# kjenike/panagram

Measured on AMD Instinct MI355X. Metric: anchored k-mers/sec building pan-kmer bitmap, higher is better.
Workload: dtype u64

## Files before the change

### panagram_amd/csrc/pg_api.hip

```cpp
#include "../../include/panagram_hip.h"
#include "pg_kernels.h"
#include "pg_guard.h"

#include <algorithm>
#include <atomic>
#include <condition_variable>
#include <cmath>
#include <cstdarg>
#include <cstdio>
#include <cstdlib>
#include <cstring>
#include <memory>
#include <mutex>
#include <string>
#include <system_error>
#include <thread>
#include <vector>

using namespace pg;

static thread_local std::string g_err;

static int fail(int code, const char *fmt, ...) {
    char buf[512];
    va_list ap;
    va_start(ap, fmt);
    vsnprintf(buf, sizeof buf, fmt, ap);
    va_end(ap);
    g_err = buf;
    return code;
}

#define HIP_TRY(expr)                                                                          \
    do {                                                                                       \
        hipError_t e_ = (expr);                                                                \
        if (e_ != hipSuccess)                                                                  \
            return fail(PG_E_HIP, "%s failed: %s (%s:%d)", #expr, hipGetErrorString(e_), __FILE__, __LINE__); \
    } while (0)

extern "C" const char *pg_last_error(void) { return g_err.c_str(); }
int pg_set_error(int code, const char *msg) {
    g_err = msg ? msg : "";
    return code;
}
extern "C" const char *pg_version(void) { return "panagram_hip 0.2 gfx950"; }
extern "C" uint32_t pg_tile_positions(void) { return (uint32_t)PROBE_TILE; }

struct pg_ctx {
    int device;
    hipStream_t own_stream;
    hipStream_t stream;
    hipStream_t aux_stream;
    std::atomic<int> refs{0};
    bool dead = false;
    struct DfSet {
        uint8_t *d_slots[2] = {nullptr, nullptr}, *d_packed[2] = {nullptr, nullptr}, *h_slots[2] = {nullptr, nullptr};
        uint32_t *d_sizes[2] = {nullptr, nullptr}, *d_offs[2] = {nullptr, nullptr}, *h_sizes[2] = {nullptr, nullptr};
        uint32_t *d_crc = nullptr, *d_hist = nullptr;
        void *d_code = nullptr;
        bool ready = false, busy = false;
    } df[4];
    std::mutex df_mu;
    std::condition_variable df_cv;
    struct RowBuf {
        uint8_t *p;
        uint64_t cap;
    };
    std::vector<RowBuf> row_cache;
    std::mutex row_mu;
};

struct SubHost {
    SubTable d;
    uint64_t count;
};

struct pg_table {
    pg_ctx *ctx;
    int k, ngenomes, ndbs;
    uint32_t m;
    bool m_pinned = false;
    uint32_t cosched = 0;
    uint64_t expected = 0;
    double load0 = 0.375;
    uint64_t first_len = 0;
    uint64_t max_len = 0;
    std::vector<SubHost> subs;
    unsigned long long *d_counters;
    unsigned long long *h_counters = nullptr;
    uint32_t *d_tile0 = nullptr;
    size_t tile0_cap = 0;
    double spill = 0;
    std::atomic<int> refs{0};
    bool dead = false;
    std::mutex write_mu;
};
#define TABLE_WRITER(t) std::lock_guard<std::mutex> writer_guard_((t)->write_mu)

struct pg_seqset {
    pg_ctx *ctx;
    uint32_t n;
    std::vector<SeqDesc> desc;
    uint64_t total_words;
    uint64_t *d_seqw;
    uint32_t *d_nmw;
    uint32_t *d_has_n;
    SeqDesc *d_desc;
    void *d_stage;
    size_t stage_cap;
    std::vector<std::string> names;
    std::atomic<int> refs{0};
    bool dead = false;
};

struct pg_result {
    pg_ctx *ctx;
    pg_table *tbl;
    const pg_seqset *seqs;
    uint32_t N;
    int k;
    uint32_t flags;
    uint32_t lowres_step = 100;
    std::vector<AnchorDesc> ad;
    std::vector<uint64_t> nrows100;
    AnchorDesc *d_ad;
    uint32_t *d_tile_contig;
    uint32_t *d_sched = nullptr;
    std::vector<uint32_t> sched_bounds;
    uint32_t ntiles;
    uint8_t *d_out1;
    uint64_t out1_bytes;
    uint64_t out1_cap = 0;
    uint8_t *d_out100;
    uint64_t out100_bytes;
    uint32_t *d_bins;
    uint64_t total_bins;
    unsigned long long *d_colsums;
    hipEvent_t ev[4];
    bool ev_ok, ev_epi;
    bool rows_valid = false;
    struct EvSet {
        hipEvent_t e[4];
        bool probe, epi;
    };
    std::vector<EvSet> ev_hist, ev_free;
    struct Chunk {
        uint32_t s0, s1, r0, nr, tiles;
    };
    std::vector<Chunk> chunks;
    uint2 *d_ranges = nullptr;
    bool chunks_ready = false;
    std::vector<hipEvent_t> chunk_ev;
    size_t hist_skip = 0;
    double probe_ms_sum = 0, epi_ms_sum = 0;
    uint32_t probe_runs = 0, epi_runs = 0;
    int fuse_state = 0;
    uint32_t *d_tile_hist = nullptr, *d_tile_cs = nullptr;
    uint2 *d_small = nullptr;
    uint32_t n_small = 0, small_tiles = 0;
    uint32_t fused_runs = 0;
};
static constexpr size_t EV_RING = 128;

static constexpr uint32_t MAX_PROBE = 512;
static constexpr double GROW_AT = 0.55;
#ifndef PG_INLINE_LAYOUT
#define PG_INLINE_LAYOUT 1
#endif
static constexpr double TARGET_LOAD = 0.375;
static constexpr double HARD_LOAD = 0.85;

static int use_device(const pg_ctx *c) {
    HIP_TRY(hipSetDevice(c->device));
    return PG_OK;
}

extern "C" int pg_ctx_create(int device_id, pg_ctx **out) {
    PG_API_BEGIN
    if (!out) return fail(PG_E_INVALID, "pg_ctx_create: out is NULL");
    int n = 0;
    hipError_t e = hipGetDeviceCount(&n);
    if (e != hipSuccess || n == 0)
        return fail(PG_E_HIP, "no HIP device visible (%s); libpanagram_hip has no CPU fallback",
                    e == hipSuccess ? "device count 0" : hipGetErrorString(e));
    if (device_id < 0 || device_id >= n) return fail(PG_E_INVALID, "device %d out of range (0..%d)", device_id, n - 1);
    HIP_TRY(hipSetDevice(device_id));
    pg_ctx *c = new pg_ctx();
    c->device = device_id;
    hipError_t se = hipStreamCreateWithFlags(&c->own_stream, hipStreamNonBlocking);
    if (se != hipSuccess) {
        delete c;
        return fail(PG_E_HIP, "hipStreamCreate failed: %s", hipGetErrorString(se));
    }
    c->stream = c->own_stream;
    se = hipStreamCreateWithFlags(&c->aux_stream, hipStreamNonBlocking);
    if (se != hipSuccess) {
        hipStreamDestroy(c->own_stream);
        delete c;
        return fail(PG_E_HIP, "hipStreamCreate failed: %s", hipGetErrorString(se));
    }
    hipError_t pe = preload_table_kernels();
    if (pe == hipSuccess) pe = preload_anchor_kernels();
    if (pe == hipSuccess) pe = preload_rows_kernels();
    if (pe == hipSuccess) pe = preload_deflate_kernels();
    if (pe != hipSuccess) {
        hipStreamDestroy(c->aux_stream);
        hipStreamDestroy(c->own_stream);
        delete c;
        return fail(PG_E_HIP, "loading the gfx950 kernels failed: %s (is this an MI355X?)", hipGetErrorString(pe));
    }
    *out = c;
    return PG_OK;
    PG_API_END
}

static void df_free_buffers(pg_ctx::DfSet &d);
static void ctx_free(pg_ctx *c) {
    hipSetDevice(c->device);
    hipStreamSynchronize(c->stream);
    hipStreamSynchronize(c->aux_stream);
    for (auto &b : c->row_cache) hipFree(b.p);
    c->row_cache.clear();
    for (auto &d : c->df) df_free_buffers(d);
    hipStreamDestroy(c->aux_stream);
    hipStreamDestroy(c->own_stream);
    delete c;
}
static void ctx_release(pg_ctx *c) {
    if (--c->refs == 0 && c->dead) ctx_free(c);
}

static constexpr uint64_t ROW_CACHE_MIN = 1ull << 30;
static void row_cache_trim(pg_ctx *c) {
    std::lock_guard<std::mutex> lk(c->row_mu);
    for (auto &b : c->row_cache) hipFree(b.p);
    c->row_cache.clear();
}
static hipError_t row_alloc(pg_ctx *c, uint64_t bytes, uint8_t **out, uint64_t *cap) {
    {
        std::lock_guard<std::mutex> lk(c->row_mu);
        for (size_t i = 0; i < c->row_cache.size(); ++i)
            if (c->row_cache[i].cap >= bytes && c->row_cache[i].cap <= 2 * bytes) {
                *out = c->row_cache[i].p;
                *cap = c->row_cache[i].cap;
                c->row_cache.erase(c->row_cache.begin() + (long)i);
                return hipSuccess;
            }
    }
    hipError_t e = hipMalloc(reinterpret_cast<void **>(out), bytes);
    if (e != hipSuccess) {
        (void)hipGetLastError();
        row_cache_trim(c);
        e = hipMalloc(reinterpret_cast<void **>(out), bytes);
    }
    *cap = bytes;
    return e;
}
static void row_free(pg_ctx *c, uint8_t *p, uint64_t cap) {
    if (!p) return;
    if (cap >= ROW_CACHE_MIN && !c->dead) {
        std::lock_guard<std::mutex> lk(c->row_mu);
        if (c->row_cache.size() < 2) {
            c->row_cache.push_back({p, cap});
            return;
        }
    }
    hipFree(p);
}

extern "C" int pg_host_alloc(pg_ctx *c, uint64_t nbytes, void **out) {
    PG_API_BEGIN
    if (!c || !out) return fail(PG_E_INVALID, "pg_host_alloc: NULL argument");
    if (int r = use_device(c)) return r;
    *out = nullptr;
    hipError_t e = hipHostMalloc(out, std::max<uint64_t>(nbytes, 1), hipHostMallocDefault);
    if (e != hipSuccess) {
        (void)hipGetLastError();
        *out = nullptr;
        return fail(PG_E_HIP, "hipHostMalloc(%llu bytes) failed: %s", (unsigned long long)nbytes, hipGetErrorString(e));
    }
    return PG_OK;
    PG_API_END
}

extern "C" int pg_host_free(pg_ctx *c, void *p) {
    PG_API_BEGIN
    if (!c) return fail(PG_E_INVALID, "ctx is NULL");
    if (!p) return PG_OK;
    if (int r = use_device(c)) return r;
    HIP_TRY(hipHostFree(p));
    return PG_OK;
    PG_API_END
// ... 1672 lines not shown
        return fail(PG_E_HIP, "pg_seqset_slice: %s", hipGetErrorString(e));
    }
    *out = s;
    return PG_OK;
    PG_API_END
}

extern "C" uint32_t pg_seqset_ncontigs(const pg_seqset *s) { return s ? s->n : 0; }

extern "C" int pg_seqset_contig(const pg_seqset *s, uint32_t idx, const char **name, uint64_t *len) {
    PG_API_BEGIN
    if (!s) return fail(PG_E_INVALID, "seqset is NULL");
    if (idx >= s->n) return fail(PG_E_INVALID, "contig %u out of range", idx);
    if (name) *name = idx < s->names.size() ? s->names[idx].c_str() : "";
    if (len) *len = s->desc[idx].len;
    return PG_OK;
    PG_API_END
}

extern "C" int pg_seqset_describe(const pg_seqset *s, uint64_t *lens, char *names, uint64_t names_cap, uint64_t *names_bytes) {
    PG_API_BEGIN
    if (!s) return fail(PG_E_INVALID, "seqset is NULL");
    uint64_t need = 0;
    for (uint32_t i = 0; i < s->n; ++i) {
        if (lens) lens[i] = s->desc[i].len;
        need += (i < s->names.size() ? s->names[i].size() : 0) + 1;
    }
    if (names_bytes) *names_bytes = need;
    if (names) {
        if (names_cap < need) return fail(PG_E_INVALID, "pg_seqset_describe: %llu bytes of names, room for %llu", (unsigned long long)need, (unsigned long long)names_cap);
        char *p = names;
        for (uint32_t i = 0; i < s->n; ++i) {
            if (i < s->names.size()) {
                memcpy(p, s->names[i].data(), s->names[i].size());
                p += s->names[i].size();
            }
            *p++ = 0;
        }
    }
    return PG_OK;
    PG_API_END
}

extern "C" int pg_seqset_unpack(const pg_seqset *s, uint32_t idx, char *out) {
    PG_API_BEGIN
    if (!s || !out) return fail(PG_E_INVALID, "pg_seqset_unpack: NULL argument");
    if (idx >= s->n) return fail(PG_E_INVALID, "contig %u out of range", idx);
    if (int r = use_device(s->ctx)) return r;
    const SeqDesc &d = s->desc[idx];
    const uint64_t nw = (d.len + 31) / 32;
    std::vector<uint64_t> w(nw);
    std::vector<uint32_t> nm(nw);
    if (nw) {
        HIP_TRY(hipMemcpyAsync(w.data(), s->d_seqw + d.seq_off, nw * 8, hipMemcpyDeviceToHost, s->ctx->stream));
        HIP_TRY(hipMemcpyAsync(nm.data(), s->d_nmw + d.seq_off, nw * 4, hipMemcpyDeviceToHost, s->ctx->stream));
        HIP_TRY(hipStreamSynchronize(s->ctx->stream));
    }
    for (uint64_t i = 0; i < d.len; ++i)
        out[i] = ((nm[i >> 5] >> (i & 31)) & 1u) ? 'N' : "ACGT"[(w[i >> 5] >> (2 * (i & 31))) & 3u];
    return PG_OK;
    PG_API_END
}

extern "C" uint64_t pg_seqset_total_kmers(const pg_seqset *s, int k) {
    uint64_t t = 0;
    if (s)
        for (auto &d : s->desc)
            if (d.len >= (uint64_t)k) t += d.len - k + 1;
    return t;
}

static TableDesc make_desc(const pg_table *t) {
    TableDesc T;
    memset(&T, 0, sizeof T);
    T.nsub = (uint32_t)t->subs.size();
    for (uint32_t i = 0; i < T.nsub; ++i) T.sub[i] = t->subs[i].d;
    T.ndbs = t->ndbs;
    T.k = t->k;
    T.ngenomes = t->ngenomes;
    return T;
}

struct ResultGeom {
    uint32_t lowres_step = 100;
    uint64_t max_bin_len = 200000;
    uint32_t min_bin_count = 100;
};

static int result_create(pg_ctx *ctx, pg_table *t, int k, uint32_t N, const pg_seqset *sq, uint32_t flags,
                         const ResultGeom &geo, pg_result **out) {
    if (ctx != sq->ctx) return fail(PG_E_INVALID, "table / context and seqset belong to different contexts");
    if (geo.lowres_step < 1 || geo.max_bin_len < 1 || geo.min_bin_count < 1)
        return fail(PG_E_INVALID, "lowres_step, max_bin_len and min_bin_count must be >= 1");
    if (int r = use_device(ctx)) return r;
    const uint32_t nbytes = (N + 7) / 8;
    pg_result *r = new pg_result();
    r->ctx = ctx;
    r->tbl = t;
    r->seqs = sq;
    r->N = N;
    r->k = k;
    if (t) ++t->refs;
    else ++ctx->refs;
    ++const_cast<pg_seqset *>(sq)->refs;
    r->flags = flags;
    r->lowres_step = geo.lowres_step;
    r->d_ad = nullptr;
    r->d_tile_contig = nullptr;
    r->d_out1 = r->d_out100 = nullptr;
    r->d_bins = nullptr;
    r->d_colsums = nullptr;
    r->ev_ok = r->ev_epi = false;
    for (auto &e : r->ev) e = nullptr;
    uint64_t o1 = 0, o100 = 0, bins = 0, tiles = 0;
    std::vector<uint32_t> tile_contig;
    for (uint32_t c = 0; c < sq->n; ++c) {
        const uint64_t len = sq->desc[c].len;
        const uint64_t nk = len >= (uint64_t)k ? len - k + 1 : 0;
        if (nk > 0xFFFFFFF0ull) {
            pg_result_destroy(r);
            return fail(PG_E_INVALID, "contig %u has %llu k-mers; contigs must stay below 2^32 (as in KMC)", c, (unsigned long long)nk);
        }
        AnchorDesc a;
        a.nkmers = (uint32_t)nk;
        uint64_t binlen = geo.max_bin_len;
        if (nk / binlen < geo.min_bin_count) binlen = nk / geo.min_bin_count;
        if (binlen == 0) binlen = 1;
        a.binlen = (uint32_t)binlen;
        a.nbins = (uint32_t)((nk + binlen - 1) / binlen);
        a.out_off = o1;
        a.out100_off = o100;
        a.bin_off = bins;
        a.tile0 = (uint32_t)tiles;
        const uint64_t n100 = (nk + geo.lowres_step - 1) / geo.lowres_step;
        r->nrows100.push_back(n100);
        o1 += (nk * nbytes + 15) & ~15ull;
        o100 += n100 * nbytes;
        bins += a.nbins;
        const uint64_t nt = (nk + PROBE_TILE - 1) / PROBE_TILE;
        for (uint64_t i = 0; i < nt; ++i) tile_contig.push_back(c);
        tiles += nt;
        r->ad.push_back(a);
    }
    if (tiles > 0x7FFFFFFFull) {
        pg_result_destroy(r);
        return fail(PG_E_INVALID, "too many tiles in one launch");
    }
    r->ntiles = (uint32_t)tiles;
    r->out1_bytes = o1;
    r->out100_bytes = o100;
    r->total_bins = bins;
    hipStream_t st = ctx->stream;
    hipError_t e;
    if ((e = hipMalloc(reinterpret_cast<void **>(&r->d_ad), std::max<size_t>(1, r->ad.size()) * sizeof(AnchorDesc))) == hipSuccess &&
        (e = hipMalloc(reinterpret_cast<void **>(&r->d_tile_contig), std::max<size_t>(1, tile_contig.size()) * 4)) == hipSuccess &&
        (e = row_alloc(ctx, (flags & PG_ANCHOR_COLUMNS_ONLY) ? 16 : std::max<uint64_t>(16, o1) + 16, &r->d_out1, &r->out1_cap)) == hipSuccess &&
        (e = hipMalloc(reinterpret_cast<void **>(&r->d_out100), std::max<uint64_t>(16, o100))) == hipSuccess &&
        (e = hipMalloc(reinterpret_cast<void **>(&r->d_bins), std::max<uint64_t>(1, bins) * (N + 1) * 4)) == hipSuccess &&
        (e = hipMalloc(reinterpret_cast<void **>(&r->d_colsums), std::max<size_t>(1, r->ad.size()) * N * 8)) == hipSuccess) {
        if (!r->ad.empty())
            e = hipMemcpyAsync(r->d_ad, r->ad.data(), r->ad.size() * sizeof(AnchorDesc), hipMemcpyHostToDevice, st);
        if (e == hipSuccess && !tile_contig.empty())
            e = hipMemcpyAsync(r->d_tile_contig, tile_contig.data(), tile_contig.size() * 4, hipMemcpyHostToDevice, st);
        if (e == hipSuccess && !t) e = hipMemsetAsync(r->d_out1, 0, std::max<uint64_t>(16, o1), st);
        if (e == hipSuccess) e = hipStreamSynchronize(st);
    }
    if (e != hipSuccess) {
        pg_result_destroy(r);
        return fail(PG_E_HIP, "result allocation failed: %s", hipGetErrorString(e));
    }
    *out = r;
    return PG_OK;
}

extern "C" int pg_result_create(pg_table *t, const pg_seqset *sq, uint32_t flags, pg_result **out) {
    PG_API_BEGIN
    if (!t || !sq || !out) return fail(PG_E_INVALID, "pg_result_create: NULL argument");
    return result_create(t->ctx, t, t->k, (uint32_t)t->ngenomes, sq, flags, ResultGeom(), out);
    PG_API_END
}

extern "C" int pg_result_create_ex(pg_table *t, const pg_seqset *sq, uint32_t flags, uint32_t lowres_step,
                                   uint64_t max_bin_len, uint32_t min_bin_count, pg_result **out) {
    PG_API_BEGIN
    if (!t || !sq || !out) return fail(PG_E_INVALID, "pg_result_create_ex: NULL argument");
    ResultGeom g;
    g.lowres_step = lowres_step;
    g.max_bin_len = max_bin_len;
    g.min_bin_count = min_bin_count;
    return result_create(t->ctx, t, t->k, (uint32_t)t->ngenomes, sq, flags, g, out);
    PG_API_END
}

extern "C" int pg_result_create_rows(pg_ctx *ctx, int k, int ngenomes, const pg_seqset *sq, uint32_t flags,
                                     uint32_t lowres_step, uint64_t max_bin_len, uint32_t min_bin_count, pg_result **out) {
    PG_API_BEGIN
    if (!ctx || !sq || !out) return fail(PG_E_INVALID, "pg_result_create_rows: NULL argument");
    if (k < 1 || k > 32) return fail(PG_E_INVALID, "k=%d unsupported (1..32)", k);
    if (ngenomes < 1) return fail(PG_E_INVALID, "ngenomes must be >= 1");
    ResultGeom g;
    g.lowres_step = lowres_step;
    g.max_bin_len = max_bin_len;
    g.min_bin_count = min_bin_count;
    return result_create(ctx, nullptr, k, (uint32_t)ngenomes, sq, flags | PG_ANCHOR_ROWS_ONLY, g, out);
    PG_API_END
}

extern "C" int pg_result_destroy(pg_result *r) {
    PG_API_BEGIN
    if (!r) return PG_OK;
    hipSetDevice(r->ctx->device);
    hipStreamSynchronize(r->ctx->stream);
    hipStreamSynchronize(r->ctx->aux_stream);
    hipFree(r->d_ad);
    hipFree(r->d_tile_contig);
    row_free(r->ctx, r->d_out1, r->out1_cap);
    hipFree(r->d_out100);
    hipFree(r->d_bins);
    hipFree(r->d_colsums);
    if (r->d_sched) hipFree(r->d_sched);
    if (r->d_ranges) hipFree(r->d_ranges);
    if (r->d_tile_hist) hipFree(r->d_tile_hist);
    if (r->d_tile_cs) hipFree(r->d_tile_cs);
    if (r->d_small) hipFree(r->d_small);
    for (auto e : r->chunk_ev) hipEventDestroy(e);
    for (auto *v : {&r->ev_hist, &r->ev_free})
        for (auto &s : *v)
            for (auto &e : s.e)
                if (e) hipEventDestroy(e);
    pg_table *t = r->tbl;
    pg_ctx *c = r->ctx;
    pg_seqset *sq = const_cast<pg_seqset *>(r->seqs);
    delete r;
    if (t) table_release(t);
    else ctx_release(c);
    seqset_release(sq);
    return PG_OK;
    PG_API_END
}

static int build_chunks(pg_result *r, const uint32_t *sched) {
    r->chunks.clear();
    r->chunks_ready = true;
    if (r->d_ranges) {
        hipFree(r->d_ranges);
        r->d_ranges = nullptr;
    }
    const char *env = getenv("PG_RUN_CHUNKS");
    const uint32_t nbytes = (r->N + 7) / 8;
    uint32_t K = env ? (uint32_t)atoi(env) : ((nbytes == 8 && r->ntiles >= (4u << 20)) ? 16u : 1u);
    const char *mt = getenv("PG_CHUNK_MIN_TILES");
    K = std::min(K, r->ntiles / std::max(1u, mt ? (uint32_t)atoi(mt) : 32768u));
    if (K < 2) return PG_OK;
    std::vector<uint2> ranges;
    for (uint32_t c = 0; c < K; ++c) {
        pg_result::Chunk ch;
        ch.s0 = (uint32_t)((uint64_t)r->ntiles * c / K);
        ch.s1 = (uint32_t)((uint64_t)r->ntiles * (c + 1) / K);
        ch.r0 = (uint32_t)ranges.size();
        ch.tiles = ch.s1 - ch.s0;
        if (!sched) {
            ranges.push_back(make_uint2(ch.s0, ch.s1));
        } else {
            std::vector<uint2> runs;
            for (uint32_t i = ch.s0; i < ch.s1; ++i) {
                if (!runs.empty() && runs.back().y == sched[i]) ++runs.back().y;
                else runs.push_back(make_uint2(sched[i], sched[i] + 1));
            }
            std::sort(runs.begin(), runs.end(), [](const uint2 &a, const uint2 &b) { return a.x < b.x; });
            for (const uint2 &u : runs) {
                if (ranges.size() > ch.r0 && ranges.back().y == u.x) ranges.back().y = u.y;
                else ranges.push_back(u);
            }
        }
        ch.nr = (uint32_t)ranges.size() - ch.r0;
        if (ch.nr > 512) {
            r->chunks.clear();
            return PG_OK;
        }
        r->chunks.push_back(ch);
    }
    HIP_TRY(hipMalloc(reinterpret_cast<void **>(&r->d_ranges), ranges.size() * sizeof(uint2)));
    HIP_TRY(hipMemcpy(r->d_ranges, ranges.data(), ranges.size() * sizeof(uint2), hipMemcpyHostToDevice));
    while (r->chunk_ev.size() < r->chunks.size()) {
        hipEvent_t e;
        HIP_TRY(hipEventCreateWithFlags(&e, hipEventDisableTiming));
        r->chunk_ev.push_back(e);
    }
    return PG_OK;
}

static int coschedule(pg_result *r, const uint32_t *contig_group, uint32_t piece_tiles, const uint32_t *range_first,
                      uint32_t nranges, const uint32_t *contig_class = nullptr) {
    if (int e = use_device(r->ctx)) return e;
    hipStream_t st = r->ctx->stream;
    HIP_TRY(hipStreamSynchronize(st));
    HIP_TRY(hipStreamSynchronize(r->ctx->aux_stream));
    if (r->d_sched) {
        hipFree(r->d_sched);
        r->d_sched = nullptr;
    }
    r->sched_bounds.clear();
    r->chunks.clear();
    r->chunks_ready = false;
    if (!contig_group || r->ntiles == 0) return PG_OK;
    const bool auto_piece = piece_tiles == 0;
    const size_t nc = r->ad.size();
    std::vector<uint32_t> firsts;
    if (range_first && nranges) {
        for (uint32_t i = 0; i < nranges; ++i) {
            if (range_first[i] >= nc || (i && range_first[i] <= range_first[i - 1]) || (!i && range_first[0] != 0))
                return fail(PG_E_INVALID, "pg_result_coschedule_ranges: range starts must begin at contig 0 and increase");
            firsts.push_back(range_first[i]);
        }
    } else {
        firsts.push_back(0);
    }
    firsts.push_back((uint32_t)nc);
    struct Piece {
        double at;
        uint32_t g, first;
    };
    std::vector<uint32_t> sched;
    sched.reserve(r->ntiles);
    std::vector<std::vector<uint32_t>> members;
    if (contig_class) {
        std::vector<std::pair<uint32_t, uint32_t>> byclass;
        for (size_t c = 0; c < nc; ++c) byclass.emplace_back(contig_class[c], (uint32_t)c);
        std::stable_sort(byclass.begin(), byclass.end(), [](auto &x, auto &y) { return x.first < y.first; });
        for (size_t i = 0; i < byclass.size(); ++i) {
            if (i == 0 || byclass[i].first != byclass[i - 1].first) members.emplace_back();
            members.back().push_back(byclass[i].second);
        }
        r->sched_bounds.push_back(0);
    } else {
        for (size_t ri = 0; ri + 1 < firsts.size(); ++ri) {
            members.emplace_back();
            for (uint32_t c = firsts[ri]; c < firsts[ri + 1]; ++c) members.back().push_back(c);
            r->sched_bounds.push_back(r->ad[firsts[ri]].tile0);
        }
    }
    for (const auto &mem : members) {
        uint32_t ngroups = 0;
        for (uint32_t c : mem) ngroups = std::max(ngroups, contig_group[c] + 1);
        std::vector<std::vector<uint32_t>> tiles(ngroups);
        for (uint32_t c : mem) {
            const uint32_t nt = (uint32_t)(((uint64_t)r->ad[c].nkmers + PROBE_TILE - 1) / PROBE_TILE);
            for (uint32_t i = 0; i < nt; ++i) tiles[contig_group[c]].push_back(r->ad[c].tile0 + i);
        }
        if (auto_piece) piece_tiles = ngroups <= 32 ? 64u : std::max(8u, 512u / ngroups);
        std::vector<Piece> pieces;
        for (uint32_t g = 0; g < ngroups; ++g) {
            const size_t np = (tiles[g].size() + piece_tiles - 1) / piece_tiles;
            for (size_t i = 0; i < np; ++i) pieces.push_back({(double)i / (double)np, g, (uint32_t)(i * piece_tiles)});
        }
        std::stable_sort(pieces.begin(), pieces.end(), [](const Piece &x, const Piece &y) { return x.at < y.at; });
        for (const Piece &p : pieces) {
            const size_t end = std::min<size_t>(tiles[p.g].size(), (size_t)p.first + piece_tiles);
            for (size_t i = p.first; i < end; ++i) sched.push_back(tiles[p.g][i]);
        }
    }
    r->sched_bounds.push_back(r->ntiles);
    if (sched.size() != r->ntiles) return fail(PG_E_INVALID, "internal: schedule does not cover the tiles");
    HIP_TRY(hipMalloc(reinterpret_cast<void **>(&r->d_sched), (size_t)r->ntiles * 4));
    HIP_TRY(hipMemcpyAsync(r->d_sched, sched.data(), (size_t)r->ntiles * 4, hipMemcpyHostToDevice, st));
    HIP_TRY(hipStreamSynchronize(st));
    if (!(r->flags & PG_ANCHOR_ROWS_ONLY)) return build_chunks(r, sched.data());
    return PG_OK;
}

extern "C" int pg_result_coschedule(pg_result *r, const uint32_t *contig_group, uint32_t piece_tiles) {
    PG_API_BEGIN
    if (!r) return fail(PG_E_INVALID, "result is NULL");
    return coschedule(r, contig_group, piece_tiles, nullptr, 0);
    PG_API_END
}

extern "C" int pg_result_coschedule_classes(pg_result *r, const uint32_t *contig_group, const uint32_t *contig_class,
                                            uint32_t piece_tiles) {
    PG_API_BEGIN
    if (!r) return fail(PG_E_INVALID, "result is NULL");
    if (contig_group && !contig_class) return fail(PG_E_INVALID, "pg_result_coschedule_classes: contig_class is NULL");
    return coschedule(r, contig_group, piece_tiles, nullptr, 0, contig_class);
    PG_API_END
}

extern "C" int pg_result_coschedule_ranges(pg_result *r, const uint32_t *contig_group, uint32_t piece_tiles,
                                           const uint32_t *range_first_contig, uint32_t nranges) {
    PG_API_BEGIN
    if (!r) return fail(PG_E_INVALID, "result is NULL");
    return coschedule(r, contig_group, piece_tiles, range_first_contig, nranges);
    PG_API_END
}

static int enqueue_epilogue(pg_result *r, hipStream_t st) {
    const uint32_t N = r->N;
    HIP_TRY(hipMemsetAsync(r->d_bins, 0, std::max<uint64_t>(1, r->total_bins) * (N + 1) * 4, st));
    HIP_TRY(hipMemsetAsync(r->d_colsums, 0, std::max<size_t>(1, r->ad.size()) * N * 8, st));
    const uint32_t kflags = (r->flags & PG_ANCHOR_COLSUMS) | (r->lowres_step == 100 ? 0u : 2u);
    HIP_TRY(launch_rows_epilogue(st, N, r->d_ad, r->d_tile_contig, r->ntiles, r->d_out1, r->d_out100, r->d_bins,
                                 r->d_colsums, kflags));
    if (r->lowres_step != 100)
        HIP_TRY(launch_lowres(st, N, r->d_ad, r->d_tile_contig, r->ntiles, r->d_out1, r->d_out100, r->lowres_step));
    return PG_OK;
}

static bool fuse_enabled() {
    const char *e = getenv("PG_FUSE_STATS");
    return e && *e == '1';
}
static bool fuse_table_ok(const TableDesc &T, uint32_t N) {
    return T.nsub == 1 && T.ngenomes == N && !(T.sub[0].layout == LAYOUT_SLOTS && T.sub[0].slots != 8);
}
static int prepare_fuse(pg_result *r, const TableDesc &T) {
    if (r->fuse_state) return PG_OK;
    r->fuse_state = -1;
    const uint32_t nbytes = (r->N + 7) / 8;
    if (!fuse_rows_ok(nbytes) || !fuse_table_ok(T, r->N)) return PG_OK;
    std::vector<uint2> small;
    uint64_t small_tiles = 0, fused_tiles = 0;
    for (const AnchorDesc &a : r->ad) {
        const uint32_t nt = (uint32_t)(((uint64_t)a.nkmers + PROBE_TILE - 1) / PROBE_TILE);
        if (!nt) continue;
        if (a.binlen >= (uint32_t)PROBE_TILE) {
            fused_tiles += nt;
            continue;
        }
        small_tiles += nt;
        if (!small.empty() && small.back().y == a.tile0) small.back().y = a.tile0 + nt;
        else small.push_back(make_uint2(a.tile0, a.tile0 + nt));
    }
    if (!fused_tiles || small.size() > 16384) return PG_OK;
    const size_t hb = (size_t)r->ntiles * fuse_hist_words(r->N) * 4, cb = (size_t)r->ntiles * fuse_cs_words(r->N) * 4;
    if (hipMalloc(reinterpret_cast<void **>(&r->d_tile_hist), hb) != hipSuccess || hipMalloc(reinterpret_cast<void **>(&r->d_tile_cs), cb) != hipSuccess ||
        (!small.empty() && hipMalloc(reinterpret_cast<void **>(&r->d_small), small.size() * sizeof(uint2)) != hipSuccess)) {
        (void)hipGetLastError();
        if (r->d_tile_hist) hipFree(r->d_tile_hist);
        if (r->d_tile_cs) hipFree(r->d_tile_cs);
        r->d_tile_hist = r->d_tile_cs = nullptr;
        return PG_OK;
    }
    if (!small.empty()) HIP_TRY(hipMemcpy(r->d_small, small.data(), small.size() * sizeof(uint2), hipMemcpyHostToDevice));
    r->n_small = (uint32_t)small.size();
    r->small_tiles = (uint32_t)small_tiles;
    r->fuse_state = 1;
    return PG_OK;
}
static FuseArgs fuse_args(const pg_result *r) {
    FuseArgs fa;
    fa.out100 = r->lowres_step == 100 ? r->d_out100 : nullptr;
    fa.tile_hist = r->d_tile_hist;
    fa.tile_cs = r->d_tile_cs;
    fa.ngenomes = r->N;
    fa.hw = fuse_hist_words(r->N);
    fa.csw = fuse_cs_words(r->N);
    return fa;
}
static int enqueue_fused_epilogue(pg_result *r, hipStream_t st, const FuseArgs &fa) {
    const uint32_t N = r->N;
    HIP_TRY(hipMemsetAsync(r->d_bins, 0, std::max<uint64_t>(1, r->total_bins) * (N + 1) * 4, st));
    HIP_TRY(hipMemsetAsync(r->d_colsums, 0, std::max<size_t>(1, r->ad.size()) * N * 8, st));
    HIP_TRY(launch_tile_reduce(st, fa, r->d_ad, r->d_tile_contig, r->ntiles, r->d_bins, r->d_colsums, (r->flags & PG_ANCHOR_COLSUMS) ? 1u : 0u));
    const uint32_t kflags = (r->flags & PG_ANCHOR_COLSUMS) | (r->lowres_step == 100 ? 0u : 2u);
    if (r->n_small)
        HIP_TRY(launch_rows_epilogue(st, N, r->d_ad, r->d_tile_contig, r->ntiles, r->d_out1, r->d_out100, r->d_bins, r->d_colsums, kflags,
                                     r->d_small, r->n_small, r->small_tiles));
    if (r->lowres_step != 100)
        HIP_TRY(launch_lowres(st, N, r->d_ad, r->d_tile_contig, r->ntiles, r->d_out1, r->d_out100, r->lowres_step));
    return PG_OK;
}

static int join_result(pg_result *r) {
    if (r->ev_epi) HIP_TRY(hipStreamWaitEvent(r->ctx->stream, r->ev[3], 0));
    return PG_OK;
}

static int fold_timing(pg_result *r, const pg_result::EvSet &s) {
    HIP_TRY(hipEventSynchronize(s.e[s.epi ? 3 : 1]));
    float a = 0, b = 0;
    if (s.probe) {
        HIP_TRY(hipEventElapsedTime(&a, s.e[0], s.e[1]));
        r->probe_ms_sum += a;
        ++r->probe_runs;
    }
    if (s.epi) {
        HIP_TRY(hipEventElapsedTime(&b, s.e[2], s.e[3]));
        r->epi_ms_sum += b;
        ++r->epi_runs;
    }
    return PG_OK;
}

static int next_events(pg_result *r, bool probe) {
    if (r->ev_hist.size() >= EV_RING) {
        if (r->hist_skip) --r->hist_skip;
        else if (int e = fold_timing(r, r->ev_hist.front())) return e;
        r->ev_free.push_back(r->ev_hist.front());
        r->ev_hist.erase(r->ev_hist.begin());
    }
    pg_result::EvSet s;
    if (!r->ev_free.empty()) {
        s = r->ev_free.back();
        r->ev_free.pop_back();
    } else {
        for (auto &e : s.e) {
            e = nullptr;
            HIP_TRY(hipEventCreate(&e));
        }
    }
    s.probe = probe;
    s.epi = false;
    r->ev_hist.push_back(s);
    for (int i = 0; i < 4; ++i) r->ev[i] = s.e[i];
    return PG_OK;
}

static int contig_tiles(const pg_result *r, uint32_t first, uint32_t n, uint32_t *t0, uint32_t *nt) {
    if ((uint64_t)first + n > r->ad.size()) return fail(PG_E_INVALID, "contigs %u..%u out of range (the result has %zu)", first, first + n, r->ad.size());
    if (n == 0) {
        *t0 = *nt = 0;
        return PG_OK;
    }
    const AnchorDesc &a = r->ad[first], &z = r->ad[first + n - 1];
    *t0 = a.tile0;
    *nt = z.tile0 + (uint32_t)(((uint64_t)z.nkmers + PROBE_TILE - 1) / PROBE_TILE) - a.tile0;
    return PG_OK;
}

static bool sched_covers(const pg_result *r, uint32_t t0, uint32_t nt) {
    if (!r->d_sched) return false;
    const auto &b = r->sched_bounds;
    return std::binary_search(b.begin(), b.end(), t0) && std::binary_search(b.begin(), b.end(), t0 + nt);
}

static int run_chunks(pg_result *r, const TableDesc &T) {
    hipStream_t st = r->ctx->stream, aux = r->ctx->aux_stream;
    if (const char *e = getenv("PG_CHUNK_SAME_STREAM"); e && *e == '1') aux = st;
    const uint32_t N = r->N;
    const uint32_t kflags = (r->flags & PG_ANCHOR_COLSUMS) | (r->lowres_step == 100 ? 0u : 2u);
    HIP_TRY(hipEventRecord(r->ev[0], st));
    for (size_t c = 0; c < r->chunks.size(); ++c) {
        const pg_result::Chunk &ch = r->chunks[c];
        HIP_TRY(launch_anchor(st, T, r->seqs->d_seqw, r->seqs->d_nmw, r->seqs->d_has_n, r->seqs->d_desc, r->d_ad, r->d_tile_contig,
                              r->d_sched, ch.s0, ch.s1 - ch.s0, r->d_out1, r->out1_bytes, 0));
        HIP_TRY(hipEventRecord(r->chunk_ev[c], st));
        HIP_TRY(hipStreamWaitEvent(aux, r->chunk_ev[c], 0));
        if (c == 0) {
            HIP_TRY(hipEventRecord(r->ev[2], aux));
            HIP_TRY(hipMemsetAsync(r->d_bins, 0, std::max<uint64_t>(1, r->total_bins) * (N + 1) * 4, aux));
            HIP_TRY(hipMemsetAsync(r->d_colsums, 0, std::max<size_t>(1, r->ad.size()) * N * 8, aux));
        }
        HIP_TRY(launch_rows_epilogue(aux, N, r->d_ad, r->d_tile_contig, r->ntiles, r->d_out1, r->d_out100, r->d_bins, r->d_colsums,
                                     kflags, r->d_ranges + ch.r0, ch.nr, ch.tiles));
    }
    HIP_TRY(hipEventRecord(r->ev[1], st));
    if (r->lowres_step != 100)
        HIP_TRY(launch_lowres(aux, N, r->d_ad, r->d_tile_contig, r->ntiles, r->d_out1, r->d_out100, r->lowres_step));
    HIP_TRY(hipEventRecord(r->ev[3], aux));
    r->ev_ok = r->ev_epi = true;
    r->ev_hist.back().epi = true;
    return PG_OK;
}

static int anchor_run(pg_result *r, uint32_t tile_base, uint32_t ntiles, bool whole, uint32_t columns_width = 0,
                      void *d_columns = nullptr) {
    pg_table *t = r->tbl;
    if (!t) return fail(PG_E_INVALID, "this result is a rows container (pg_result_create_rows): it has no table to probe");
    if (int e = use_device(r->ctx)) return e;
    hipStream_t st = r->ctx->stream, aux = r->ctx->aux_stream;
    if (int e = join_result(r)) return e;
    if (int e = next_events(r, true)) return e;
    TableDesc T = make_desc(t);
    const bool stats = whole && !columns_width && !(r->flags & PG_ANCHOR_ROWS_ONLY);
    bool fuse = false;
    if (stats && fuse_enabled()) {
        if (int e = prepare_fuse(r, T)) return e;
        fuse = r->fuse_state == 1 && fuse_table_ok(T, r->N);
    }
    if (stats && !fuse) {
        if (!r->chunks_ready)
            if (int e = build_chunks(r, nullptr)) return e;
        if (r->chunks.size() > 1) return run_chunks(r, T);
    }
    const FuseArgs fa = fuse_args(r);
    HIP_TRY(hipEventRecord(r->ev[0], st));
    HIP_TRY(launch_anchor(st, T, r->seqs->d_seqw, r->seqs->d_nmw, r->seqs->d_has_n, r->seqs->d_desc, r->d_ad,
                          r->d_tile_contig, sched_covers(r, tile_base, ntiles) ? r->d_sched : nullptr, tile_base, ntiles,
                          columns_width ? static_cast<uint8_t *>(d_columns) : r->d_out1, r->out1_bytes, columns_width, fuse ? &fa : nullptr));
    HIP_TRY(hipEventRecord(r->ev[1], st));
    r->ev_ok = true;
    r->ev_epi = false;
    if (stats) {
        HIP_TRY(hipStreamWaitEvent(aux, r->ev[1], 0));
        HIP_TRY(hipEventRecord(r->ev[2], aux));
        if (fuse) {
            if (int e = enqueue_fused_epilogue(r, aux, fa)) return e;
            ++r->fused_runs;
        } else if (int e = enqueue_epilogue(r, aux)) return e;
        HIP_TRY(hipEventRecord(r->ev[3], aux));
        r->ev_epi = true;
        r->ev_hist.back().epi = true;
    }
    return PG_OK;
}

extern "C" int pg_anchor_run(pg_result *r) {
    PG_API_BEGIN
    if (!r) return fail(PG_E_INVALID, "result is NULL");
    if (r->flags & PG_ANCHOR_COLUMNS_ONLY) return fail(PG_E_INVALID, "a PG_ANCHOR_COLUMNS_ONLY result has no rows: use pg_anchor_run_columns_range");
    return anchor_run(r, 0, r->ntiles, true);
    PG_API_END
}

extern "C" int pg_anchor_run_range(pg_result *r, uint32_t first_contig, uint32_t ncontigs) {
    PG_API_BEGIN
    if (!r) return fail(PG_E_INVALID, "result is NULL");
    if (r->flags & PG_ANCHOR_COLUMNS_ONLY) return fail(PG_E_INVALID, "a PG_ANCHOR_COLUMNS_ONLY result has no rows: use pg_anchor_run_columns_range");
    if (!(r->flags & PG_ANCHOR_ROWS_ONLY)) return fail(PG_E_INVALID, "pg_anchor_run_range needs a PG_ANCHOR_ROWS_ONLY result");
    uint32_t t0, nt;
    if (int e = contig_tiles(r, first_contig, ncontigs, &t0, &nt)) return e;
    return anchor_run(r, t0, nt, false);
    PG_API_END
}

extern "C" int pg_result_columns_direct(const pg_result *r, uint32_t width) {
    PG_API_BEGIN
    if (!r || !r->tbl) return 0;
    const pg_table *t = r->tbl;
    return t->subs.size() == 1 && t->subs[0].d.layout == LAYOUT_SLOTS && t->subs[0].d.W == 1 && t->subs[0].d.slots == 8 &&
           t->ngenomes <= 8 && width <= 8 && (int)width >= t->ngenomes;
    PG_API_END
}

extern "C" int pg_anchor_run_columns_range(pg_result *r, uint32_t first_contig, uint32_t ncontigs, uint32_t width, void *d_dst) {
    PG_API_BEGIN
    if (!r || !d_dst) return fail(PG_E_INVALID, "pg_anchor_run_columns_range: NULL argument");
    if (!pg_result_columns_direct(r, width))
        return fail(PG_E_INVALID, "pg_anchor_run_columns_range: needs a table of up to 8 genomes (8-slot lines) and width in ngenomes..8");
    uint32_t t0, nt;
    if (int e = contig_tiles(r, first_contig, ncontigs, &t0, &nt)) return e;
    return anchor_run(r, t0, nt, false, width, d_dst);
    PG_API_END
}

extern "C" int pg_result_timing(pg_result *r, float *probe_ms, float *epilogue_ms) {
    PG_API_BEGIN
    if (!r) return fail(PG_E_INVALID, "result is NULL");
    if (!r->ev_ok) return fail(PG_E_INVALID, "pg_anchor_run has not been called on this result");
    if (int e = use_device(r->ctx)) return e;
    HIP_TRY(hipEventSynchronize(r->ev[r->ev_epi ? 3 : 1]));
    float a = 0, b = 0;
    HIP_TRY(hipEventElapsedTime(&a, r->ev[0], r->ev[1]));
    if (r->ev_epi) HIP_TRY(hipEventElapsedTime(&b, r->ev[2], r->ev[3]));
    if (probe_ms) *probe_ms = a;
    if (epilogue_ms) *epilogue_ms = b;
    return PG_OK;
    PG_API_END
}

extern "C" int pg_result_fused_runs(const pg_result *r, uint32_t *n) {
    PG_API_BEGIN
    if (!r || !n) return fail(PG_E_INVALID, "pg_result_fused_runs: NULL argument");
    *n = r->fused_runs;
    return PG_OK;
    PG_API_END
}

extern "C" int pg_result_timing_reset(pg_result *r) {
    PG_API_BEGIN
    if (!r) return fail(PG_E_INVALID, "result is NULL");
    while (r->ev_hist.size() > 1) {
        r->ev_free.push_back(r->ev_hist.front());
        r->ev_hist.erase(r->ev_hist.begin());
    }
    r->hist_skip = r->ev_hist.size();
    r->probe_ms_sum = r->epi_ms_sum = 0;
    r->probe_runs = r->epi_runs = 0;
    return PG_OK;
    PG_API_END
}

extern "C" int pg_result_timing_mean(pg_result *r, double *probe_ms, double *epilogue_ms, uint32_t *nruns) {
    PG_API_BEGIN
    if (!r) return fail(PG_E_INVALID, "result is NULL");
    if (int e = use_device(r->ctx)) return e;
    const double a0 = r->probe_ms_sum, b0 = r->epi_ms_sum;
    const uint32_t pn0 = r->probe_runs, en0 = r->epi_runs;
    int rc = PG_OK;
    for (size_t i = r->hist_skip; i < r->ev_hist.size() && !rc; ++i) rc = fold_timing(r, r->ev_hist[i]);
    if (!rc) {
        if (probe_ms) *probe_ms = r->probe_runs ? r->probe_ms_sum / r->probe_runs : 0.0;
        if (epilogue_ms) *epilogue_ms = r->epi_runs ? r->epi_ms_sum / r->epi_runs : 0.0;
        if (nruns) *nruns = r->probe_runs;
    }
    r->probe_ms_sum = a0;
    r->epi_ms_sum = b0;
    r->probe_runs = pn0;
    r->epi_runs = en0;
    return rc;
    PG_API_END
}

extern "C" uint64_t pg_result_columns_bytes(const pg_result *r, uint32_t width) {
    return r ? (uint64_t)r->ntiles * (PROBE_TILE / 8) * width : 0;
}

extern "C" uint64_t pg_result_columns_bytes_range(const pg_result *r, uint32_t width, uint32_t first_contig, uint32_t ncontigs) {
    uint32_t t0, nt;
    if (!r || contig_tiles(r, first_contig, ncontigs, &t0, &nt)) return 0;
    return (uint64_t)nt * (PROBE_TILE / 8) * width;
}

extern "C" int pg_result_extract_columns_range(pg_result *r, uint32_t g0, uint32_t width, uint32_t first_contig,
                                               uint32_t ncontigs, void *d_dst) {
    PG_API_BEGIN
    if (!r || !d_dst) return fail(PG_E_INVALID, "pg_result_extract_columns: NULL argument");
    if (!r->ev_ok && !r->rows_valid) return fail(PG_E_INVALID, "the result holds no rows yet");
    uint32_t t0, nt;
    if (int e = contig_tiles(r, first_contig, ncontigs, &t0, &nt)) return e;
    if (int e = use_device(r->ctx)) return e;
    HIP_TRY(launch_cols_extract(r->ctx->stream, r->N, r->d_ad, r->d_tile_contig, t0, nt, r->d_out1, g0, width, d_dst));
    return PG_OK;
    PG_API_END
}

extern "C" int pg_result_extract_columns(pg_result *r, uint32_t g0, uint32_t width, void *d_dst) {
    PG_API_BEGIN
    if (!r) return fail(PG_E_INVALID, "pg_result_extract_columns: NULL argument");
    return pg_result_extract_columns_range(r, g0, width, 0, (uint32_t)r->ad.size(), d_dst);
    PG_API_END
}

extern "C" int pg_result_merge_columns_range(pg_result *r, const void *d_src, uint32_t part0, uint32_t nparts, uint32_t per,
                                             uint32_t first_contig, uint32_t ncontigs, int accumulate,
                                             uint64_t part_stride_bytes) {
    PG_API_BEGIN
    if (!r || !d_src) return fail(PG_E_INVALID, "pg_result_merge_columns: NULL argument");
    if (per == 0 || nparts == 0) return fail(PG_E_INVALID, "pg_result_merge_columns: empty partition");
    uint32_t t0, nt;
    if (int e = contig_tiles(r, first_contig, ncontigs, &t0, &nt)) return e;
    const uint64_t own = (uint64_t)nt * (PROBE_TILE / 8) * per;
    if (part_stride_bytes == 0) part_stride_bytes = own;
    if (part_stride_bytes < own || part_stride_bytes % 8) return fail(PG_E_INVALID, "pg_result_merge_columns_range: bad block stride");
    if (int e = use_device(r->ctx)) return e;
    if (int e = join_result(r)) return e;
    HIP_TRY(launch_cols_merge(r->ctx->stream, r->N, r->d_ad, r->d_tile_contig, t0, nt, r->d_out1, d_src, part0, nparts,
                              part_stride_bytes / 8, per, accumulate ? 1u : 0u));
    r->rows_valid = true;
    return PG_OK;
    PG_API_END
}

extern "C" int pg_result_merge_columns(pg_result *r, const void *d_src, uint32_t nparts, uint32_t per) {
    PG_API_BEGIN
    if (!r) return fail(PG_E_INVALID, "pg_result_merge_columns: NULL argument");
    return pg_result_merge_columns_range(r, d_src, 0, nparts, per, 0, (uint32_t)r->ad.size(), 0, 0);
    PG_API_END
}

extern "C" int pg_rows_epilogue(pg_result *r) {
    PG_API_BEGIN
    if (!r) return fail(PG_E_INVALID, "result is NULL");
    if (int e = use_device(r->ctx)) return e;
    if (int e = join_result(r)) return e;
    hipStream_t st = r->ctx->stream;
    if (int e = next_events(r, false)) return e;
    HIP_TRY(hipEventRecord(r->ev[0], st));
    HIP_TRY(hipEventRecord(r->ev[1], st));
    HIP_TRY(hipEventRecord(r->ev[2], st));
    if (int e = enqueue_epilogue(r, st)) return e;
    HIP_TRY(hipEventRecord(r->ev[3], st));
    r->ev_ok = true;
    r->ev_epi = true;
    r->ev_hist.back().epi = true;
    return PG_OK;
    PG_API_END
}

static constexpr uint32_t CRC_TAB_WORDS = DF_CRC_TAB_WORDS;
static const uint32_t *crc_tables_host() {
    static uint32_t tab[CRC_TAB_WORDS];
    static std::once_flag once;
    std::call_once(once, [] {
        for (uint32_t i = 0; i < 256; ++i) {
            uint32_t c = i;
            for (int k = 0; k < 8; ++k) c = (c & 1) ? 0xEDB88320u ^ (c >> 1) : c >> 1;
            tab[i] = c;
        }
        for (uint32_t k = 1; k < 4; ++k)
            for (uint32_t b = 0; b < 256; ++b) tab[256 * k + b] = (tab[256 * (k - 1) + b] >> 8) ^ tab[tab[256 * (k - 1) + b] & 255u];
        uint32_t *T0 = tab + 1024;
        for (uint32_t k = 0; k < 4; ++k)
            for (uint32_t b = 0; b < 256; ++b) {
                uint32_t s = b << (8 * k);
                for (uint32_t z = 0; z < DF_CHUNK_BYTES; ++z) s = tab[s & 255u] ^ (s >> 8);
                T0[256 * k + b] = s;
            }
        for (uint32_t j = 1; j < DF_CRC_LEVELS; ++j) {
            const uint32_t *P = tab + 1024 + 1024 * (j - 1);
            uint32_t *T = tab + 1024 + 1024 * j;
            auto apply = [&](uint32_t x) { return P[x & 255u] ^ P[256 + ((x >> 8) & 255u)] ^ P[512 + ((x >> 16) & 255u)] ^ P[768 + (x >> 24)]; };
            for (uint32_t k = 0; k < 4; ++k)
                for (uint32_t b = 0; b < 256; ++b) T[256 * k + b] = apply(apply(b << (8 * k)));
        }
    });
    return tab;
}

#ifndef PG_DF_BATCH
#define PG_DF_BATCH 1024
#endif
static constexpr uint32_t DF_BATCH = PG_DF_BATCH;

static pg_ctx::DfSet *df_acquire(pg_ctx *ctx) {
    std::unique_lock<std::mutex> lk(ctx->df_mu);
    for (;;) {
        for (auto &d : ctx->df)
            if (!d.busy) {
                d.busy = true;
                return &d;
            }
        ctx->df_cv.wait(lk);
    }
}
static void df_release(pg_ctx *ctx, pg_ctx::DfSet *D) {
    {
        std::lock_guard<std::mutex> lk(ctx->df_mu);
        D->busy = false;
    }
    ctx->df_cv.notify_one();
}
static void df_free_buffers(pg_ctx::DfSet &d) {
    for (int i = 0; i < 2; ++i) {
        if (d.d_slots[i]) hipFree(d.d_slots[i]);
        if (d.d_packed[i]) hipFree(d.d_packed[i]);
        if (d.d_sizes[i]) hipFree(d.d_sizes[i]);
        if (d.d_offs[i]) hipFree(d.d_offs[i]);
        if (d.h_slots[i]) hipHostFree(d.h_slots[i]);
        if (d.h_sizes[i]) hipHostFree(d.h_sizes[i]);
        d.d_slots[i] = d.d_packed[i] = d.h_slots[i] = nullptr;
        d.d_sizes[i] = d.d_offs[i] = d.h_sizes[i] = nullptr;
    }
    if (d.d_crc) hipFree(d.d_crc);
    if (d.d_hist) hipFree(d.d_hist);
    if (d.d_code) hipFree(d.d_code);
    d.d_crc = d.d_hist = nullptr;
    d.d_code = nullptr;
    d.ready = false;
}

static int write_bgzf_gpu(pg_result *r, const uint8_t *src, const std::vector<std::pair<uint64_t, uint64_t>> &segs_in,
                          uint64_t total, uint32_t row, const char *gz_path, const char *gzi_path) {
    static const unsigned char EOF_BLOCK[28] = {0x1f, 0x8b, 0x08, 0x04, 0, 0, 0, 0, 0, 0xff, 0x06, 0x00, 0x42, 0x43,
                                                0x02, 0x00, 0x1b, 0x00, 0x03, 0x00, 0, 0, 0, 0, 0, 0, 0, 0};
    pg_ctx *ctx = r->ctx;
    const uint64_t nblocks = (total + 65279) / 65280;
    std::vector<PaySeg> segs;
    uint64_t l = 0;
    for (auto &sg : segs_in) {
        segs.push_back({l, sg.first});
        l += sg.second;
    }
    segs.push_back({total, 0});
    FILE *f = fopen(gz_path, "wb");
    if (!f) return fail(PG_E_IO, "cannot open %s for writing", gz_path);
    pg_ctx::DfSet *D = df_acquire(ctx);
    hipStream_t cs = nullptr;
    PaySeg *d_segs = nullptr;
    hipEvent_t done[2] = {nullptr, nullptr}, copied[2] = {nullptr, nullptr};
    hipError_t e = hipStreamCreateWithFlags(&cs, hipStreamNonBlocking);
    auto ok = [&](hipError_t x) {
        if (e == hipSuccess) e = x;
        return e == hipSuccess;
    };
    if (!D->ready) {
        ok(hipMalloc(reinterpret_cast<void **>(&D->d_crc), CRC_TAB_WORDS * 4));
        ok(hipMalloc(reinterpret_cast<void **>(&D->d_hist), DF_HIST_WORDS * 4));
        ok(hipMalloc(&D->d_code, DF_CODE_BYTES));
        for (int i = 0; i < 2; ++i) {
            ok(hipMalloc(reinterpret_cast<void **>(&D->d_slots[i]), (size_t)DF_BATCH * 65536));
            ok(hipMalloc(reinterpret_cast<void **>(&D->d_packed[i]), (size_t)DF_BATCH * 65536));
            ok(hipMalloc(reinterpret_cast<void **>(&D->d_sizes[i]), (size_t)DF_BATCH * 4));
            ok(hipMalloc(reinterpret_cast<void **>(&D->d_offs[i]), (size_t)(DF_BATCH + 1) * 4));
            ok(hipHostMalloc(reinterpret_cast<void **>(&D->h_slots[i]), (size_t)DF_BATCH * 65536, 0));
            ok(hipHostMalloc(reinterpret_cast<void **>(&D->h_sizes[i]), (size_t)(DF_BATCH + 1) * 4, 0));
        }
        if (e == hipSuccess) {
            ok(hipMemcpyAsync(D->d_crc, crc_tables_host(), CRC_TAB_WORDS * 4, hipMemcpyHostToDevice, cs));
            ok(hipStreamSynchronize(cs));
        }
        D->ready = e == hipSuccess;
        if (!D->ready) df_free_buffers(*D);
    }
    ok(hipMalloc(reinterpret_cast<void **>(&d_segs), segs.size() * sizeof(PaySeg)));
    for (int i = 0; i < 2; ++i) {
        ok(hipEventCreateWithFlags(&done[i], hipEventDisableTiming));
        ok(hipEventCreateWithFlags(&copied[i], hipEventDisableTiming));
    }
    if (e == hipSuccess) {
        ok(hipMemcpyAsync(d_segs, segs.data(), segs.size() * sizeof(PaySeg), hipMemcpyHostToDevice, cs));
        ok(hipStreamWaitEvent(cs, r->ev[r->ev_epi ? 3 : 1], 0));
    }
    if (e == hipSuccess && nblocks) ok(launch_deflate_code(cs, src, d_segs, (uint32_t)segs.size() - 1, total, row, D->d_hist, D->d_code));
    std::vector<uint64_t> coffs, uoffs;
    uint64_t cpos = 0;
    int rc = PG_OK;
    auto issue = [&](uint64_t b0, int slot) {
        const uint32_t nb = (uint32_t)std::min<uint64_t>(DF_BATCH, nblocks - b0);
        hipError_t x = hipMemsetAsync(D->d_slots[slot], 0, (size_t)nb * 65536, cs);
        if (x == hipSuccess)
            x = launch_row_deflate(cs, src, d_segs, (uint32_t)segs.size() - 1, total, b0, nb, row, D->d_crc, D->d_code, D->d_slots[slot],
                                   D->d_sizes[slot], getenv("PG_DEFLATE_FORCE_STORED") ? (uint32_t)atoi(getenv("PG_DEFLATE_FORCE_STORED")) : 0u, D->d_offs[slot], D->d_packed[slot]);
        if (x == hipSuccess)
            x = hipMemcpyAsync(D->h_sizes[slot], D->d_offs[slot], (size_t)(nb + 1) * 4, hipMemcpyDeviceToHost, cs);
        if (x == hipSuccess) x = hipEventRecord(done[slot], cs);
        return x;
    };
    if (e == hipSuccess && nblocks) ok(issue(0, 0));
    int slot = 0;
    for (uint64_t b0 = 0; e == hipSuccess && rc == PG_OK && b0 < nblocks; b0 += DF_BATCH, slot ^= 1) {
        const uint32_t nb = (uint32_t)std::min<uint64_t>(DF_BATCH, nblocks - b0);
        if (!ok(hipEventSynchronize(done[slot]))) break;
        const uint32_t *offs = D->h_sizes[slot];
        const uint32_t bytes = offs[nb];
        if (bytes < 26u * nb || bytes > nb * 65536ull) {
            rc = fail(PG_E_IO, "GPU deflate produced %u bytes for %u blocks", bytes, nb);
// ... 769 lines not shown
```

Before: 237.9 billion.

## Merge stats buffers, zero them on aux stream, run epilogue on main stream

Bins and column sums now share one allocation, so a single memset clears both instead of two. In the single-launch stats path, the zeroing is issued on the auxiliary stream so it overlaps the anchor kernel, and the epilogue runs on the main stream after an event wait, which removes the cross-stream handoff. The old side-stream behaviour stays available behind an environment variable. join_result skips the wait when the epilogue already ran on the main stream, at the cost of extra events and more complex stream bookkeeping.

Result: no change. 238.0 billion, median of 2 (+0.0%).

```diff
diff --git a/panagram_amd/csrc/pg_api.hip b/panagram_amd/csrc/pg_api.hip
--- a/panagram_amd/csrc/pg_api.hip
+++ b/panagram_amd/csrc/pg_api.hip
@@ -136,8 +136,11 @@
     uint32_t *d_bins;
     uint64_t total_bins;
     unsigned long long *d_colsums;
+    uint64_t stats_bytes = 0;
     hipEvent_t ev[4];
     bool ev_ok, ev_epi;
+    hipStream_t ev_stream = nullptr;
+    hipEvent_t ev_zero[2] = {nullptr, nullptr};
     bool rows_valid = false;
     struct EvSet {
         hipEvent_t e[4];
@@ -2116,12 +2119,14 @@
     r->total_bins = bins;
     hipStream_t st = ctx->stream;
     hipError_t e;
+    const uint64_t bins_bytes = (std::max<uint64_t>(1, bins) * (N + 1) * 4 + 7) & ~7ull;
+    r->stats_bytes = bins_bytes + std::max<size_t>(1, r->ad.size()) * N * 8;
     if ((e = hipMalloc(reinterpret_cast<void **>(&r->d_ad), std::max<size_t>(1, r->ad.size()) * sizeof(AnchorDesc))) == hipSuccess &&
         (e = hipMalloc(reinterpret_cast<void **>(&r->d_tile_contig), std::max<size_t>(1, tile_contig.size()) * 4)) == hipSuccess &&
         (e = row_alloc(ctx, (flags & PG_ANCHOR_COLUMNS_ONLY) ? 16 : std::max<uint64_t>(16, o1) + 16, &r->d_out1, &r->out1_cap)) == hipSuccess &&
         (e = hipMalloc(reinterpret_cast<void **>(&r->d_out100), std::max<uint64_t>(16, o100))) == hipSuccess &&
-        (e = hipMalloc(reinterpret_cast<void **>(&r->d_bins), std::max<uint64_t>(1, bins) * (N + 1) * 4)) == hipSuccess &&
-        (e = hipMalloc(reinterpret_cast<void **>(&r->d_colsums), std::max<size_t>(1, r->ad.size()) * N * 8)) == hipSuccess) {
+        (e = hipMalloc(reinterpret_cast<void **>(&r->d_bins), r->stats_bytes)) == hipSuccess) {
+        r->d_colsums = reinterpret_cast<unsigned long long *>(reinterpret_cast<uint8_t *>(r->d_bins) + bins_bytes);
         if (!r->ad.empty())
             e = hipMemcpyAsync(r->d_ad, r->ad.data(), r->ad.size() * sizeof(AnchorDesc), hipMemcpyHostToDevice, st);
         if (e == hipSuccess && !tile_contig.empty())
@@ -2181,13 +2186,14 @@
     row_free(r->ctx, r->d_out1, r->out1_cap);
     hipFree(r->d_out100);
     hipFree(r->d_bins);
-    hipFree(r->d_colsums);
     if (r->d_sched) hipFree(r->d_sched);
     if (r->d_ranges) hipFree(r->d_ranges);
     if (r->d_tile_hist) hipFree(r->d_tile_hist);
     if (r->d_tile_cs) hipFree(r->d_tile_cs);
     if (r->d_small) hipFree(r->d_small);
     for (auto e : r->chunk_ev) hipEventDestroy(e);
+    for (auto e : r->ev_zero)
+        if (e) hipEventDestroy(e);
     for (auto *v : {&r->ev_hist, &r->ev_free})
         for (auto &s : *v)
             for (auto &e : s.e)
@@ -2357,10 +2363,15 @@
     PG_API_END
 }
 
-static int enqueue_epilogue(pg_result *r, hipStream_t st) {
+static int zero_stats(pg_result *r, hipStream_t st) {
+    HIP_TRY(hipMemsetAsync(r->d_bins, 0, r->stats_bytes, st));
+    return PG_OK;
+}
+
+static int enqueue_epilogue(pg_result *r, hipStream_t st, bool zeroed = false) {
     const uint32_t N = r->N;
-    HIP_TRY(hipMemsetAsync(r->d_bins, 0, std::max<uint64_t>(1, r->total_bins) * (N + 1) * 4, st));
-    HIP_TRY(hipMemsetAsync(r->d_colsums, 0, std::max<size_t>(1, r->ad.size()) * N * 8, st));
+    if (!zeroed)
+        if (int e = zero_stats(r, st)) return e;
     const uint32_t kflags = (r->flags & PG_ANCHOR_COLSUMS) | (r->lowres_step == 100 ? 0u : 2u);
     HIP_TRY(launch_rows_epilogue(st, N, r->d_ad, r->d_tile_contig, r->ntiles, r->d_out1, r->d_out100, r->d_bins,
                                  r->d_colsums, kflags));
@@ -2422,8 +2433,7 @@
 }
 static int enqueue_fused_epilogue(pg_result *r, hipStream_t st, const FuseArgs &fa) {
     const uint32_t N = r->N;
-    HIP_TRY(hipMemsetAsync(r->d_bins, 0, std::max<uint64_t>(1, r->total_bins) * (N + 1) * 4, st));
-    HIP_TRY(hipMemsetAsync(r->d_colsums, 0, std::max<size_t>(1, r->ad.size()) * N * 8, st));
+    if (int e = zero_stats(r, st)) return e;
     HIP_TRY(launch_tile_reduce(st, fa, r->d_ad, r->d_tile_contig, r->ntiles, r->d_bins, r->d_colsums, (r->flags & PG_ANCHOR_COLSUMS) ? 1u : 0u));
     const uint32_t kflags = (r->flags & PG_ANCHOR_COLSUMS) | (r->lowres_step == 100 ? 0u : 2u);
     if (r->n_small)
@@ -2435,8 +2445,13 @@
 }
 
 static int join_result(pg_result *r) {
-    if (r->ev_epi) HIP_TRY(hipStreamWaitEvent(r->ctx->stream, r->ev[3], 0));
-    return PG_OK;
+    if (r->ev_epi && r->ev_stream != r->ctx->stream) HIP_TRY(hipStreamWaitEvent(r->ctx->stream, r->ev[3], 0));
+    return PG_OK;
+}
+
+static bool stats_side_stream() {
+    const char *e = getenv("PG_STATS_SIDE_STREAM");
+    return e && *e == '1';
 }
 
 static int fold_timing(pg_result *r, const pg_result::EvSet &s) {
@@ -2511,8 +2526,7 @@
         HIP_TRY(hipStreamWaitEvent(aux, r->chunk_ev[c], 0));
         if (c == 0) {
             HIP_TRY(hipEventRecord(r->ev[2], aux));
-            HIP_TRY(hipMemsetAsync(r->d_bins, 0, std::max<uint64_t>(1, r->total_bins) * (N + 1) * 4, aux));
-            HIP_TRY(hipMemsetAsync(r->d_colsums, 0, std::max<size_t>(1, r->ad.size()) * N * 8, aux));
+            if (int e = zero_stats(r, aux)) return e;
         }
         HIP_TRY(launch_rows_epilogue(aux, N, r->d_ad, r->d_tile_contig, r->ntiles, r->d_out1, r->d_out100, r->d_bins, r->d_colsums,
                                      kflags, r->d_ranges + ch.r0, ch.nr, ch.tiles));
@@ -2522,6 +2536,7 @@
         HIP_TRY(launch_lowres(aux, N, r->d_ad, r->d_tile_contig, r->ntiles, r->d_out1, r->d_out100, r->lowres_step));
     HIP_TRY(hipEventRecord(r->ev[3], aux));
     r->ev_ok = r->ev_epi = true;
+    r->ev_stream = aux;
     r->ev_hist.back().epi = true;
     return PG_OK;
 }
@@ -2547,6 +2562,20 @@
         if (r->chunks.size() > 1) return run_chunks(r, T);
     }
     const FuseArgs fa = fuse_args(r);
+    const bool side = stats && stats_side_stream();
+    bool zeroed = false;
+    if (stats && !fuse && !side) {
+        const char *zi = getenv("PG_STATS_ZERO_INLINE");
+        zeroed = !(zi && *zi == '1');
+    }
+    if (zeroed) {
+        for (auto &e : r->ev_zero)
+            if (!e) HIP_TRY(hipEventCreateWithFlags(&e, hipEventDisableTiming));
+        HIP_TRY(hipEventRecord(r->ev_zero[0], st));
+        HIP_TRY(hipStreamWaitEvent(aux, r->ev_zero[0], 0));
+        if (int e = zero_stats(r, aux)) return e;
+        HIP_TRY(hipEventRecord(r->ev_zero[1], aux));
+    }
     HIP_TRY(hipEventRecord(r->ev[0], st));
     HIP_TRY(launch_anchor(st, T, r->seqs->d_seqw, r->seqs->d_nmw, r->seqs->d_has_n, r->seqs->d_desc, r->d_ad,
                           r->d_tile_contig, sched_covers(r, tile_base, ntiles) ? r->d_sched : nullptr, tile_base, ntiles,
@@ -2555,14 +2584,17 @@
     r->ev_ok = true;
     r->ev_epi = false;
     if (stats) {
-        HIP_TRY(hipStreamWaitEvent(aux, r->ev[1], 0));
-        HIP_TRY(hipEventRecord(r->ev[2], aux));
+        const hipStream_t es = side ? aux : st;
+        if (side) HIP_TRY(hipStreamWaitEvent(aux, r->ev[1], 0));
+        else if (zeroed) HIP_TRY(hipStreamWaitEvent(st, r->ev_zero[1], 0));
+        HIP_TRY(hipEventRecord(r->ev[2], es));
         if (fuse) {
-            if (int e = enqueue_fused_epilogue(r, aux, fa)) return e;
+            if (int e = enqueue_fused_epilogue(r, es, fa)) return e;
             ++r->fused_runs;
-        } else if (int e = enqueue_epilogue(r, aux)) return e;
-        HIP_TRY(hipEventRecord(r->ev[3], aux));
+        } else if (int e = enqueue_epilogue(r, es, zeroed)) return e;
+        HIP_TRY(hipEventRecord(r->ev[3], es));
         r->ev_epi = true;
+        r->ev_stream = es;
         r->ev_hist.back().epi = true;
     }
     return PG_OK;
@@ -2736,6 +2768,7 @@
     HIP_TRY(hipEventRecord(r->ev[3], st));
     r->ev_ok = true;
     r->ev_epi = true;
+    r->ev_stream = st;
     r->ev_hist.back().epi = true;
     return PG_OK;
     PG_API_END
```
